# nkwangyh/CubemapSLAM

Measured on AMD Instinct MI355X. Metric: frames/sec (extract+match+localBA) on Lafida cam0, higher is better.
Workload: dtype u8 (extract/match), f64 (BA)

## Files before the change

### cubemapslam_amd/csrc/cms_api_area.hip

```cpp
#include <mutex>
#include <vector>

static int cms_area_grid_attr(int device) {
  static std::mutex mu;
  static bool done[64] = {false};
  std::lock_guard<std::mutex> lk(mu);
  if (device >= 0 && device < 64 && !done[device]) {
    HIPCHK(hipFuncSetAttribute((const void*)k_area_grid, hipFuncAttributeMaxDynamicSharedMemorySize, (CMS_AREA_MAXKP + 1) * 8));
    done[device] = true;
  }
  return CMS_OK;
}
static int cms_area_reserve(cms_ctx* c) {
  if (c->d_area_sorted) return CMS_OK;
  if (c->g.kp_cap > CMS_AREA_MAXKP) return cms_fail(CMS_ERR_UNSUPPORTED, "frame grid: more than 16383 key points per frame");
  { const int rca = cms_area_grid_attr(c->device); if (rca) return rca; }
  const size_t B = (size_t)c->max_batch;
  HIPCHK(hipMalloc((void**)&c->d_area_sorted, B * c->g.kp_cap * sizeof(uint16_t)));
  HIPCHK(hipMalloc((void**)&c->d_area_cell_start, B * (CMS_AREA_CELLS + 1) * sizeof(int)));
  HIPCHK(hipMalloc((void**)&c->d_area_nvalid, B * sizeof(int)));
  return CMS_OK;
}

static int cms_area_tmp_reserve(cms_ctx* c, int nq) {
  if ((size_t)nq <= c->area_tmp_cap) return CMS_OK;
  if (c->d_area_tmp) hipFree(c->d_area_tmp);
  c->d_area_tmp = nullptr; c->area_tmp_cap = 0;
  const size_t cap = (size_t)nq + (size_t)nq / 4 + 1024;
  HIPCHK(hipMalloc((void**)&c->d_area_tmp, cap * CMS_AREA_TMP * sizeof(int)));
  c->area_tmp_cap = cap;
  return CMS_OK;
}
static int cms_area_bsum_reserve(cms_ctx* c, int nblk) {
  if (nblk <= c->area_bsum_cap) return CMS_OK;
  if (c->d_area_bsum) hipFree(c->d_area_bsum);
  c->d_area_bsum = nullptr; c->area_bsum_cap = 0;
  HIPCHK(hipMalloc((void**)&c->d_area_bsum, (size_t)(nblk + 64) * sizeof(int)));
  c->area_bsum_cap = nblk + 64;
  return CMS_OK;
}

extern "C" int cms_area_set_keypoints(cms_ctx* c, int b, int n, const cms_keypoint* kps) {
  if (!c || b < 0 || b >= c->max_batch || n < 0 || n > c->g.kp_cap || (n > 0 && !kps)) return cms_fail(CMS_ERR_ARG, "cms_area_set_keypoints: bad argument");
  HIPCHK(hipSetDevice(c->device));
  if (n > 0) HIPCHK(hipMemcpyAsync(c->d_kps + (size_t)b * c->g.kp_cap, kps, (size_t)n * sizeof(cms_keypoint), hipMemcpyHostToDevice, c->stream));
  HIPCHK(hipMemcpyAsync(c->d_kp_cnt + b, &n, sizeof(int), hipMemcpyHostToDevice, c->stream));
  HIPCHK(hipStreamSynchronize(c->stream));
  return CMS_OK;
}

extern "C" int cms_area_grid(cms_ctx* c, int B) {
  if (!c || B < 1 || B > c->max_batch) return cms_fail(CMS_ERR_ARG, "cms_area_grid: bad batch");
  HIPCHK(hipSetDevice(c->device));
// ... 8 lines not shown
}

extern "C" int cms_features_in_area_device(cms_ctx* c, int b, int nq, const void* d_qx, const void* d_qy, const void* d_qr, const void* d_qmin,
                                           const void* d_qmax, void* d_cnt_scratch, void* d_cand_off, void* d_cand_idx, int cap, int idx_base,
                                           void* d_total) {
  if (!c || b < 0 || b >= c->area_frames || nq < 0 || cap < 0) return cms_fail(CMS_ERR_ARG, "cms_features_in_area_device: bad argument (cms_area_grid first)");
  if (nq == 0) return CMS_OK;
  HIPCHK(hipSetDevice(c->device));
  CmsAreaArgs a;
  a.kp = (const CmsKeyPoint*)c->d_kps + (size_t)b * c->g.kp_cap;
  a.sorted_idx = c->d_area_sorted + (size_t)b * c->g.kp_cap;
  a.cell_start = c->d_area_cell_start + (size_t)b * (CMS_AREA_CELLS + 1);
  a.qx = (const float*)d_qx; a.qy = (const float*)d_qy; a.qr = (const float*)d_qr; a.qmin = (const int*)d_qmin; a.qmax = (const int*)d_qmax;
  a.q_frame = nullptr; a.kp_cap = c->g.kp_cap;
  a.nq = nq; a.F = c->g.F; a.inv = (float)(3 * CMS_AREA_G) / (float)c->g.W;
  a.cnt = (int*)d_cnt_scratch; a.off = (const int*)d_cand_off; a.idx = (int*)d_cand_idx; a.cap = cap; a.idx_base = idx_base;
  hipStream_t s = c->stream;
  {
    const int nblk = (nq + 1023) / 1024, qgrid = (nq * CMS_AREA_QL + 255) / 256;
    int rcb = cms_area_bsum_reserve(c, nblk);
    if (rcb) return rcb;
    rcb = cms_area_tmp_reserve(c, nq);
    if (rcb) return rcb;
    a.tmp = c->d_area_tmp;
    hipLaunchKernelGGL(k_area_query, dim3(qgrid), dim3(256), 0, s, a, 0);
    hipLaunchKernelGGL(k_area_blocksum, dim3(nblk), dim3(1024), 0, s, (const int*)d_cnt_scratch, nq, c->d_area_bsum);
    hipLaunchKernelGGL(k_area_scan, dim3(nblk), dim3(1024), 0, s, (const int*)d_cnt_scratch, nq, (const int*)c->d_area_bsum, (int*)d_cand_off, (int*)d_total);
    hipLaunchKernelGGL(k_area_query, dim3(qgrid), dim3(256), 0, s, a, 1);
  }
  HIPCHK(hipGetLastError());
  return CMS_OK;
}

extern "C" int cms_features_in_area_batch_device(cms_ctx* c, int nq, const void* d_qframe, const void* d_qx, const void* d_qy, const void* d_qr,
                                                 const void* d_qmin, const void* d_qmax, void* d_cnt_scratch, void* d_cand_off, void* d_cand_idx,
                                                 int cap, void* d_total) {
  if (!c || nq < 0 || cap < 0 || c->area_frames < 1 || !d_qframe) return cms_fail(CMS_ERR_ARG, "cms_features_in_area_batch_device: bad argument (cms_area_grid first)");
  if (nq == 0) return CMS_OK;
  HIPCHK(hipSetDevice(c->device));
  CmsAreaArgs a;
  a.kp = (const CmsKeyPoint*)c->d_kps; a.sorted_idx = c->d_area_sorted; a.cell_start = c->d_area_cell_start;
  a.qx = (const float*)d_qx; a.qy = (const float*)d_qy; a.qr = (const float*)d_qr; a.qmin = (const int*)d_qmin; a.qmax = (const int*)d_qmax;
  a.q_frame = (const int*)d_qframe; a.kp_cap = c->g.kp_cap;
  a.nq = nq; a.F = c->g.F; a.inv = (float)(3 * CMS_AREA_G) / (float)c->g.W;
  a.cnt = (int*)d_cnt_scratch; a.off = (const int*)d_cand_off; a.idx = (int*)d_cand_idx; a.cap = cap; a.idx_base = 0;
  hipStream_t s = c->stream;
  {
    const int nblk = (nq + 1023) / 1024, qgrid = (nq * CMS_AREA_QL + 255) / 256;
    int rcb = cms_area_bsum_reserve(c, nblk);
    if (rcb) return rcb;
    rcb = cms_area_tmp_reserve(c, nq);
    if (rcb) return rcb;
    a.tmp = c->d_area_tmp;
    hipLaunchKernelGGL(k_area_query, dim3(qgrid), dim3(256), 0, s, a, 0);
    hipLaunchKernelGGL(k_area_blocksum, dim3(nblk), dim3(1024), 0, s, (const int*)d_cnt_scratch, nq, c->d_area_bsum);
    hipLaunchKernelGGL(k_area_scan, dim3(nblk), dim3(1024), 0, s, (const int*)d_cnt_scratch, nq, (const int*)c->d_area_bsum, (int*)d_cand_off, (int*)d_total);
    hipLaunchKernelGGL(k_area_query, dim3(qgrid), dim3(256), 0, s, a, 1);
  }
  HIPCHK(hipGetLastError());
  return CMS_OK;
}

extern "C" int cms_features_in_area(cms_ctx* c, int b, int nq, const float* qx, const float* qy, const float* qr, const int* qmin, const int* qmax,
                                    int* cand_off, int* cand_idx, int cap, int* total) {
  if (!c || nq < 0 || cap < 0 || !cand_off || (nq > 0 && (!qx || !qy || !qr || !qmin || !qmax))) return cms_fail(CMS_ERR_ARG, "cms_features_in_area: bad argument");
  if (b < 0 || b >= c->area_frames) return cms_fail(CMS_ERR_ARG, "cms_features_in_area: no grid for this frame (cms_area_grid first)");
  cand_off[0] = 0;
  if (total) *total = 0;
  if (nq == 0) return CMS_OK;
  HIPCHK(hipSetDevice(c->device));
  const size_t qb = (size_t)nq * 4;
  const size_t bytes = 5 * qb + qb  + (qb + 4)  + (size_t)cap * 4 + 64;
  int rc = cms_scratch(c, bytes);
  if (rc) return rc;
  uint8_t* p = (uint8_t*)c->d_match;
// ... 20 lines not shown
```

### cubemapslam_amd/csrc/cms_api_frames.hip

```cpp
#include <chrono>
#include <thread>
#include <hip/hip_runtime.h>
#include <math.h>
#include <stdio.h>
#include <stdlib.h>
#include <string.h>
#include <algorithm>
#include <string>
#include <vector>
#include "../../include/cubemapslam_hip.h"
#include "cms_types.h"
#include "orb_pattern.inc"

static bool cms_cu_mask_from_env(uint32_t* words, int* n_words) {
  const char* v = getenv("CMS_CTX_CU_MASK");
  if (!v || !*v) return false;
  int n = 0;
  while (*v && n < 8) {
    char* end = nullptr;
    words[n++] = (uint32_t)strtoul(v, &end, 16);
    if (end == v) return false;
    v = *end == ',' ? end + 1 : end;
    if (*end && *end != ',') return false;
  }
// ... 30 lines not shown
  CmsGeom g;
  float scale[CMS_MAX_LEVELS], inv_scale[CMS_MAX_LEVELS], sigma2[CMS_MAX_LEVELS], inv_sigma2[CMS_MAX_LEVELS];
  hipStream_t stream = nullptr;
  int fstride = 0;
  size_t fish_pitch = 0;
  int lut_stride = 0, mstride = 0;
  bool have_mask = false;
  int dirty_frames = 0;
  uint8_t* d_fish = nullptr; uint32_t* d_lut = nullptr; uint8_t* d_pyr = nullptr; uint8_t* d_mask = nullptr;
  CmsResizeTab* d_tab = nullptr; float* d_pattern = nullptr;
  uint32_t* d_cand = nullptr; uint16_t* d_node = nullptr; int* d_cand_cnt = nullptr; int* d_overflow = nullptr;
  uint32_t* d_qt_out = nullptr; int* d_qt_cnt = nullptr;
  uint32_t* d_cell_cand = nullptr; int* d_cell_cnt = nullptr;
  int* d_cells_all = nullptr; int* d_cells_nz = nullptr; int n_cells_all = 0, n_cells_nz = 0;
  uint16_t* d_area_sorted = nullptr; int* d_area_cell_start = nullptr; int* d_area_nvalid = nullptr; int area_frames = 0;
  int* d_area_bsum = nullptr; int area_bsum_cap = 0;
  int* d_area_tmp = nullptr; size_t area_tmp_cap = 0;
  uint8_t* h_fish_stage = nullptr; int fish_stage_frames = 0;
  hipStream_t copy_stream = nullptr; hipEvent_t ev_upload_done = nullptr, ev_remap_done = nullptr;
  bool upload_pending = false, remap_recorded = false;
  int dist_bounds_scaled = 0;
  hipEvent_t ev_block = nullptr; int last_batch = 0;
  hipEvent_t ev_extracted = nullptr; bool extracted_recorded = false;
  uint8_t* h_stage = nullptr; size_t h_stage_bytes = 0;
  CmsKeyPoint* d_kps = nullptr; uint32_t* d_aux = nullptr; uint8_t* d_desc = nullptr; int* d_kp_cnt = nullptr;
  uint32_t* d_order = nullptr; uint32_t* d_aux_sorted = nullptr; int* d_walk_cnt = nullptr; float* d_rays = nullptr;
  void* d_match = nullptr; size_t match_bytes = 0;
  bool prof = false;
  bool desc_spatial = false;
  hipEvent_t ev[8] = {nullptr, nullptr, nullptr, nullptr, nullptr, nullptr, nullptr, nullptr};
  size_t fast_lds = 0, qt_lds = 0;
// ... 68 lines not shown
    }
    out[d].s = (short)s;
    out[d].a0 = cms_sat_short((1.f - f) * 2048);
    out[d].a1 = cms_sat_short(f * 2048);
    out[d].pad = 0;
  }
}

static size_t align_up(size_t v, size_t a) { return (v + a - 1) / a * a; }

static void cms_ctx_free(cms_ctx* c) {
  if (!c) return;
  hipSetDevice(c->device);
  void* ptrs[] = {c->d_fish, c->d_lut, c->d_pyr, c->d_mask, c->d_tab, c->d_pattern, c->d_cand, c->d_node, c->d_cand_cnt,
                  c->d_overflow, c->d_qt_out, c->d_qt_cnt, c->d_kps, c->d_aux, c->d_order, c->d_aux_sorted, c->d_desc, c->d_kp_cnt, c->d_match, c->d_cell_cand,
                  c->d_cell_cnt, c->d_cells_all, c->d_cells_nz, c->d_area_sorted, c->d_area_cell_start, c->d_area_nvalid, c->d_area_bsum, c->d_area_tmp, c->d_walk_cnt, c->d_rays};
  for (void* p : ptrs) if (p) hipFree(p);
  if (c->h_fish_stage) (void)hipHostFree(c->h_fish_stage);
  if (c->h_stage) (void)hipHostFree(c->h_stage);
  for (int i = 0; i < 8; ++i) if (c->ev[i]) hipEventDestroy(c->ev[i]);
  if (c->ev_extracted) hipEventDestroy(c->ev_extracted);
  if (c->ev_block) hipEventDestroy(c->ev_block);
  if (c->ev_upload_done) hipEventDestroy(c->ev_upload_done);
  if (c->ev_remap_done) hipEventDestroy(c->ev_remap_done);
  if (c->copy_stream) hipStreamDestroy(c->copy_stream);
  if (c->stream) hipStreamDestroy(c->stream);
  delete c;
}

extern "C" int cms_ctx_create(cms_ctx** out, int device, const cms_camera* cam, const cms_orb_params* orb, int max_batch) {
  if (!out || !cam || !orb || max_batch < 1) return cms_fail(CMS_ERR_ARG, "cms_ctx_create: bad argument");
// ... 661 lines not shown
```

### cubemapslam_amd/csrc/cms_api_tri.hip

```cpp
#include <algorithm>
#include <cmath>
#include <cstdlib>
#include <cstring>
#include <memory>
#include <mutex>
#include <vector>

namespace {
inline float tri_h_small(const float* a, const float* b, int bs) {
  float t = a[0] * b[0];
  t = t + a[1] * b[bs];
  t = t + a[2] * b[2 * bs];
  return t;
}
void tri_h_e12(const float* R1w, const float* t1w, const float* R2w, const float* t2w, float* E12) {
  float R12[9], M[9], t12[3];
  for (int r = 0; r < 3; ++r)
    for (int c = 0; c < 3; ++c) {
      double s = 0;
      for (int k = 0; k < 3; ++k) s += (double)R1w[3 * r + k] * (double)R2w[3 * c + k];
      R12[3 * r + c] = (float)(s * 1.0);
      M[3 * r + c] = (float)(s * -1.0);
    }
  for (int r = 0; r < 3; ++r) t12[r] = (float)((double)tri_h_small(M + 3 * r, t2w, 1) * 1.0 + (double)t1w[r] * 1.0);
// ... 802 lines not shown
    const int sl = job_slot[j];
    if (sl < 0 || sl >= st->maxkf || !st->used[(size_t)sl] || mp_off[j + 1] < mp_off[j]) return cms_fail(CMS_ERR_ARG, "cms_kfstore_fuse_search: bad job");
    const CmsTriKF& k = st->h_kf[(size_t)sl];
    memcpy(&pose[15 * (size_t)j], k.Rcw, 36); memcpy(&pose[15 * (size_t)j + 9], k.tcw, 12); memcpy(&pose[15 * (size_t)j + 12], k.Ow, 12);
  }
  HIPCHK(hipSetDevice(c->device));
  HIPCHK(kfstore_order_behind_puts(st));
  hipStream_t s = c->stream;
  if (!job_set0) npts = nmp;
  const size_t n4 = (size_t)nmp * 4, j4 = (size_t)njobs * 4, p4 = (size_t)npts * 4;
  auto al = [](size_t v) { return (v + 255) & ~(size_t)255; };
  size_t o = 0;
  auto take = [&](size_t bytes) { const size_t at = o; o += al(bytes); return at; };
  const size_t o_pose = take(pose.size() * 4), o_joff = take(j4 + 4), o_jslot = take(j4), o_jset = take(j4), o_src = take(n4), o_job = take(n4), o_slot = take(n4), o_skip = take(nmp),
               o_pos = take(3 * p4), o_nrm = take(3 * p4), o_min = take(p4), o_max = take(p4), o_desc = take((size_t)npts * 32), o_qx = take(n4), o_qy = take(n4), o_qr = take(n4),
               o_qmin = take(n4), o_qmax = take(n4), o_lvl = take(n4), o_cnt = take(n4), o_off = take(n4 + 4), o_tot = take(16), o_bi = take(n4), o_bd = take(n4);
  const size_t fixed = o;
  bool direct = false;
  {
    hipPointerAttribute_t a1, a2;
    if (hipPointerGetAttributes(&a1, best_idx) == hipSuccess && hipPointerGetAttributes(&a2, best_dist) == hipSuccess)
      direct = a1.type == hipMemoryTypeHost && a2.type == hipMemoryTypeHost;
    else (void)hipGetLastError();
  }
  int cap = 64 * nmp + 1024;
  for (int attempt = 0; attempt < 2; ++attempt) {
    int rc = cms_scratch(c, fixed + al((size_t)cap * 4));
    if (rc) return rc;
    uint8_t* p = (uint8_t*)c->d_match;
    const size_t o_idx = fixed;
    HIPCHK(hipMemcpyAsync(p + o_pose, pose.data(), pose.size() * 4, hipMemcpyHostToDevice, s));
// ... 8 lines not shown
    HIPCHK(hipMemcpyAsync(p + o_desc, mp_desc, (size_t)npts * 32, hipMemcpyHostToDevice, s));
    const int* src_dev = job_set0 ? (const int*)(p + o_src) : nullptr;
    hipLaunchKernelGGL(k_fuse_expand_jobs, dim3((nmp + 255) / 256), dim3(256), 0, s, nmp, njobs, (const int*)(p + o_joff), (const int*)(p + o_jslot), (int*)(p + o_job), (int*)(p + o_slot),
                       job_set0 ? (const int*)(p + o_jset) : nullptr, job_set0 ? (int*)(p + o_src) : nullptr);
    CmsFuseArgs fa;
    fa.src = src_dev;
    fa.bounds_scaled = c->dist_bounds_scaled;
    fa.pose15 = (const float*)(p + o_pose); fa.mp_frame = (const int*)(p + o_job); fa.n = nmp; fa.skip = skip ? p + o_skip : nullptr;
    fa.P = (const float*)(p + o_pos); fa.normal = (const float*)(p + o_nrm); fa.min_dist = (const float*)(p + o_min); fa.max_dist = (const float*)(p + o_max);
    fa.th = th; fa.log_scale = std::log(c->scale[1]); fa.nlevels = c->g.nlevels; fa.F = c->g.F;
    for (int l = 0; l < 16; ++l) fa.sf[l] = l < c->g.nlevels ? c->scale[l] : 0.0f;
    fa.qx = (float*)(p + o_qx); fa.qy = (float*)(p + o_qy); fa.qr = (float*)(p + o_qr); fa.qmin = (int*)(p + o_qmin); fa.qmax = (int*)(p + o_qmax);
    fa.level = (int*)(p + o_lvl);
    hipLaunchKernelGGL(k_fuse_project, dim3((nmp + 255) / 256), dim3(256), 0, s, fa);
    CmsAreaArgs a;
    a.tmp = nullptr;
    a.kp = (const CmsKeyPoint*)st->d_kp; a.sorted_idx = st->d_sorted; a.cell_start = st->d_cell_start;
    a.qx = fa.qx; a.qy = fa.qy; a.qr = fa.qr; a.qmin = fa.qmin; a.qmax = fa.qmax;
    a.q_frame = (const int*)(p + o_slot); a.kp_cap = st->maxf;
    a.nq = nmp; a.F = c->g.F; a.inv = (float)(3 * CMS_AREA_G) / (float)c->g.W;
    a.cnt = (int*)(p + o_cnt); a.off = (const int*)(p + o_off); a.idx = (int*)(p + o_idx); a.cap = cap; a.idx_base = 0;
    {
      const int nblk = (nmp + 1023) / 1024, qgrid = (nmp * CMS_AREA_QL + 255) / 256;
      rc = cms_area_bsum_reserve(c, nblk);
      if (rc) return rc;
      hipLaunchKernelGGL(k_area_query, dim3(qgrid), dim3(256), 0, s, a, 0);
      hipLaunchKernelGGL(k_area_blocksum, dim3(nblk), dim3(1024), 0, s, (const int*)(p + o_cnt), nmp, c->d_area_bsum);
      hipLaunchKernelGGL(k_area_scan, dim3(nblk), dim3(1024), 0, s, (const int*)(p + o_cnt), nmp, (const int*)c->d_area_bsum, (int*)(p + o_off), (int*)(p + o_tot));
      hipLaunchKernelGGL(k_area_query, dim3(qgrid), dim3(256), 0, s, a, 1);
    }
    CmsFuseScanArgs sa;
    sa.cap = cap; sa.src = src_dev; sa.row_slot = (const int*)(p + o_slot); sa.maxf = st->maxf;
    sa.n = nmp; sa.qx = fa.qx; sa.qy = fa.qy; sa.level = fa.level; sa.mp_desc = (const uint4*)(p + o_desc);
    sa.cand_off = (const int*)(p + o_off); sa.cand_idx = (const int*)(p + o_idx); sa.kp = (const CmsKeyPoint*)st->d_kp; sa.t_desc = (const uint4*)st->d_desc;
    for (int l = 0; l < 16; ++l) sa.inv_sigma2[l] = l < c->g.nlevels ? c->inv_sigma2[l] : 0.0f;
    sa.best_idx = direct ? best_idx : (int*)(p + o_bi); sa.best_dist = direct ? best_dist : (int*)(p + o_bd);
    hipLaunchKernelGGL(k_fuse_scan, dim3((nmp * 8 + 255) / 256), dim3(256), 0, s, sa);
    HIPCHK(hipGetLastError());
    int tot = 0;
    HIPCHK(hipMemcpyAsync(&tot, p + o_tot, sizeof(int), hipMemcpyDeviceToHost, s));
    if (!direct) {
      HIPCHK(hipMemcpyAsync(best_idx, p + o_bi, n4, hipMemcpyDeviceToHost, s));
      HIPCHK(hipMemcpyAsync(best_dist, p + o_bd, n4, hipMemcpyDeviceToHost, s));
    }
    HIPCHK(hipStreamSynchronize(s));
// ... 30 lines not shown
```

### cubemapslam_amd/csrc/cms_area_kernels.hip

```cpp
#include <hip/hip_runtime.h>
#include <stdint.h>
#include "cms_types.h"
#include "cms_area_table.h"

#define CMS_AREA_CELLS (5 * CMS_AREA_G * CMS_AREA_G)
#define CMS_AREA_MAXKP 16383

extern "C" __global__ void __launch_bounds__(1024)
k_area_grid(const CmsKeyPoint* __restrict__ kps, const int* __restrict__ kp_cnt, int kp_cap, int F, float inv,
            uint16_t* __restrict__ sorted_idx, int* __restrict__ cell_start, int* __restrict__ n_valid_out) {
  extern __shared__ uint32_t area_lds[];
  uint32_t* keys = area_lds;
  uint32_t* sorted = area_lds + (kp_cap + 1);
  __shared__ int s_nvalid;
  const int b = blockIdx.x, tid = threadIdx.x, T = blockDim.x;
  const int n = min(kp_cnt[b], min(kp_cap, CMS_AREA_MAXKP));
  const CmsKeyPoint* kp = kps + (size_t)b * kp_cap;
  if (tid == 0) s_nvalid = 0;
  __syncthreads();
  for (int i = tid; i < n; i += T) {
    const float x = kp[i].x, y = kp[i].y;
    const double fi = (double)(x / (float)F), fj = (double)(y / (float)F);
    int f = -1;
    if (fi >= 0 && fi < 1 && fj >= 1 && fj < 2) f = 1;
// ... 27 lines not shown
  }
  const int last = nv ? (int)(sorted[nv - 1] >> 14) : -1;
  for (int cc = last + 1 + tid; cc <= CMS_AREA_CELLS; cc += T) cs[cc] = nv;
  if (tid == 0) n_valid_out[b] = nv;
}

struct CmsAreaArgs {
  const CmsKeyPoint* kp;
  const uint16_t* sorted_idx;
  const int* cell_start;
  const float* qx; const float* qy; const float* qr; const int* qmin; const int* qmax;
  const int* q_frame;
  int kp_cap;
  int nq, F; float inv;
  int* cnt;
  const int* off;
  int* idx; int cap; int idx_base;
  int* tmp;
};
#define CMS_AREA_TMP 8

#define CMS_AREA_QL 8
extern "C" __global__ void __launch_bounds__(256) k_area_query(CmsAreaArgs a, int pass) {
  const int gl = threadIdx.x & (CMS_AREA_QL - 1);
  const int q = (blockIdx.x * blockDim.x + threadIdx.x) / CMS_AREA_QL;
  const int qq = q < a.nq ? q : 0;
  const float x = a.qx[qq], y = a.qy[qq], r = a.qr[qq];
  const bool live = q < a.nq && !(r < 0.0f);
  const int minLevel = a.qmin[qq], maxLevel = a.qmax[qq];
  const bool check = (minLevel > 0) || (maxLevel >= 0);
  CmsAreaRectI rc[3];
  const int base = (pass && live) ? a.off[qq] : 0;
  bool copied = false;
  if (pass && a.tmp && live) {
    const int c = a.cnt[qq];
    if (c <= CMS_AREA_TMP) {
      if (gl < c && base + gl < a.cap) a.idx[base + gl] = a.tmp[(size_t)qq * CMS_AREA_TMP + gl];
      copied = true;
    }
  }
  const int nr = (live && !copied) ? cms_area_rects(x, y, r, a.F, a.inv, rc) : 0;
  int n = 0;
  int* tmpq = (!pass && a.tmp) ? a.tmp + (size_t)qq * CMS_AREA_TMP : nullptr;
  const int fr = a.q_frame ? a.q_frame[qq] : 0;
  const CmsKeyPoint* kp = a.kp + (size_t)fr * a.kp_cap;
  const uint16_t* sorted_idx = a.sorted_idx + (size_t)fr * a.kp_cap;
  const int* cell_start = a.cell_start + (size_t)fr * (CMS_AREA_CELLS + 1);
  const int idx_base = a.idx_base + (a.q_frame ? fr * a.kp_cap : 0);
  for (int k = 0; k < 3; ++k) {
    const bool has = k < nr;
    const int x0 = has ? max(0, rc[k].x0) : 0, x1 = has ? min(CMS_AREA_G - 1, rc[k].x1) : -1;
    const int y0 = has ? max(0, rc[k].y0) : 0, y1 = has ? min(CMS_AREA_G - 1, rc[k].y1) : -1;
    const int face = has ? rc[k].face : 0;
    const int ncol = (x1 >= x0 && y1 >= y0) ? x1 - x0 + 1 : 0;
    int maxcol = ncol;
    for (int o = 32; o > 0; o >>= 1) maxcol = max(maxcol, __shfl_xor(maxcol, o));
    for (int cb = 0; cb < maxcol; cb += CMS_AREA_QL) {
      const int ix = x0 + cb + gl;
      const bool col = cb + gl < ncol;
// ... 8 lines not shown
        const int j = sorted_idx[s];
        const CmsKeyPoint p = kp[j];
        if (check) {
          if (p.octave < minLevel) continue;
          if (maxLevel >= 0 && p.octave > maxLevel) continue;
        }
        if (fabsf(p.x - x) < r && fabsf(p.y - y) < r) {
          if (nh == 0) h0 = j; else if (nh == 1) h1 = j; else if (nh == 2) h2 = j; else if (nh == 3) h3 = j;
          ++nh;
        }
      }
      int incl = nh;
#pragma unroll
      for (int o = 1; o < CMS_AREA_QL; o <<= 1) { const int t = __shfl_up(incl, o, CMS_AREA_QL); if (gl >= o) incl += t; }
      const int tot = __shfl(incl, CMS_AREA_QL - 1, CMS_AREA_QL);
      if (tmpq && nh > 0) {
        int w = n + incl - nh;
        if (w < CMS_AREA_TMP) {
          if (nh <= 4) {
            tmpq[w] = idx_base + h0;
            if (nh > 1 && w + 1 < CMS_AREA_TMP) tmpq[w + 1] = idx_base + h1;
            if (nh > 2 && w + 2 < CMS_AREA_TMP) tmpq[w + 2] = idx_base + h2;
            if (nh > 3 && w + 3 < CMS_AREA_TMP) tmpq[w + 3] = idx_base + h3;
          } else {
            for (int s = s0; s < s1 && w < CMS_AREA_TMP; ++s) {
              const int j = sorted_idx[s];
              const CmsKeyPoint p = kp[j];
              if (check && (p.octave < minLevel || (maxLevel >= 0 && p.octave > maxLevel))) continue;
              if (fabsf(p.x - x) < r && fabsf(p.y - y) < r) { tmpq[w] = idx_base + j; ++w; }
            }
          }
        }
      }
      if (pass && nh > 0) {
        int w = base + n + incl - nh;
        if (nh <= 4) {
          if (w < a.cap) a.idx[w] = idx_base + h0;
          if (nh > 1 && w + 1 < a.cap) a.idx[w + 1] = idx_base + h1;
          if (nh > 2 && w + 2 < a.cap) a.idx[w + 2] = idx_base + h2;
          if (nh > 3 && w + 3 < a.cap) a.idx[w + 3] = idx_base + h3;
        } else {
          for (int s = s0; s < s1; ++s) {
            const int j = sorted_idx[s];
            const CmsKeyPoint p = kp[j];
            if (check && (p.octave < minLevel || (maxLevel >= 0 && p.octave > maxLevel))) continue;
            if (fabsf(p.x - x) < r && fabsf(p.y - y) < r) { if (w < a.cap) a.idx[w] = idx_base + j; ++w; }
          }
        }
      }
      n += tot;
    }
  }
  if (!pass && q < a.nq && gl == 0) a.cnt[q] = n;
}

extern "C" __global__ void __launch_bounds__(1024) k_area_blocksum(const int* __restrict__ cnt, int nq, int* __restrict__ bsum) {
  __shared__ int part[16];
  const int i = blockIdx.x * 1024 + threadIdx.x, lane = threadIdx.x & 63, wv = threadIdx.x >> 6;
  int v = i < nq ? cnt[i] : 0;
  for (int o = 32; o > 0; o >>= 1) v += __shfl_xor(v, o);
  if (lane == 0) part[wv] = v;
  __syncthreads();
  if (threadIdx.x == 0) { int t = 0; for (int w = 0; w < 16; ++w) t += part[w]; bsum[blockIdx.x] = t; }
}
extern "C" __global__ void __launch_bounds__(1024) k_area_scan(const int* __restrict__ cnt, int nq, const int* __restrict__ bsum,
                                                                int* __restrict__ off, int* __restrict__ total) {
  __shared__ int part[16];
  __shared__ int s_before;
  const int tid = threadIdx.x, lane = tid & 63, wv = tid >> 6;
  int before = 0;
  for (int b = tid; b < (int)blockIdx.x; b += 1024) before += bsum[b];
  for (int o = 32; o > 0; o >>= 1) before += __shfl_xor(before, o);
  if (lane == 0) part[wv] = before;
  __syncthreads();
  if (tid == 0) { int t = 0; for (int w = 0; w < 16; ++w) t += part[w]; s_before = t; }
  __syncthreads();
  const int i = blockIdx.x * 1024 + tid;
  const int v = i < nq ? cnt[i] : 0;
  int incl = v;
#pragma unroll
  for (int o = 1; o < 64; o <<= 1) { const int t = __shfl_up(incl, o); if (lane >= o) incl += t; }
  __syncthreads();
  if (lane == 63) part[wv] = incl;
  __syncthreads();
  int wbase = 0;
  for (int w = 0; w < wv; ++w) wbase += part[w];
  const int mine = s_before + wbase + incl;
  if (i < nq) off[i + 1] = mine;
  if (i == 0) off[0] = 0;
  if (i == nq - 1 && total) *total = mine;
}
```

### cubemapslam_amd/csrc/cms_area_table.h

```cpp
#ifndef CMS_AREA_TABLE_H
#define CMS_AREA_TABLE_H
#include <stdint.h>

#define CMS_AREA_G 50
#ifdef CMS_AREA_HOST_EMU
#include <math.h>
#define AREA_TAB static const
#define AREA_FN inline
#else
#define AREA_TAB static const __device__
#define AREA_FN __device__ __forceinline__
#endif

enum { AV_A, AV_B, AV_C, AV_D,
       AV_BO, AV_DO,
       AV_AU, AV_CU,
       AV_AN, AV_CN,
       AV_COUNT };
#define AE_Z 0
#define AE_G1 1
#define AE_GG 2
#define AE_V(v) (3 + (v))
#define AE_M(v) (3 + AV_COUNT + (v))

// ... 86 lines not shown
    else if (i >= 2 && i < 3 && j >= 1 && j < 2) face = 2;
  }
  if (face < 0) return 0;
  const int cornerX = (int)x / F * F, cornerY = (int)y / F * F;
  const float xin = x - (float)cornerX, yin = y - (float)cornerY;
  const float xs = xin - r, xe = xin + r, ys = yin - r, ye = yin + r;
  const bool xu = xs < 0, xo = xe > (float)(F - 1), yu = ys < 0, yo = ye > (float)(F - 1);
  const bool xinf = !xo && !xu, yinf = !yo && !yu;
  const float Ff = (float)F;
  int v[AV_COUNT];
  v[AV_A] = (int)floorf(xs * inv); v[AV_B] = (int)floorf(xe * inv); v[AV_C] = (int)floorf(ys * inv); v[AV_D] = (int)floorf(ye * inv);
  v[AV_BO] = (int)floorf((xe - Ff) * inv); v[AV_DO] = (int)floorf((ye - Ff) * inv);
  v[AV_AU] = (int)floorf((xs + Ff) * inv); v[AV_CU] = (int)floorf((ys + Ff) * inv);
  v[AV_AN] = (int)floorf((-xs) * inv); v[AV_CN] = (int)floorf((-ys) * inv);
  const CmsAreaCase* cs;
  CmsAreaCase inside;
  if (xinf && yinf) {
    inside.n = 1;
    inside.r[0].face = (int8_t)face; inside.r[0].x0 = vA; inside.r[0].x1 = vB; inside.r[0].y0 = vC; inside.r[0].y1 = vD;
    cs = &inside;
  } else if (xinf) {
    cs = &kAreaXin[face][yo ? 0 : 1];
  } else if (yinf) {
    cs = &kAreaYin[face][xo ? 0 : 1];
  } else {
    int k;
    if (xo && yo) k = 0; else if (xu && yo) k = 1; else if (xo && yu) k = 2; else k = 3;
    cs = &kAreaCorner[face][k];
  }
  auto ev = [&](int e) -> int {
    if (e == AE_Z) return 0;
    if (e == AE_G1) return CMS_AREA_G - 1;
    if (e == AE_GG) return CMS_AREA_G;
    if (e < 3 + AV_COUNT) return v[e - 3];
    return CMS_AREA_G - v[e - 3 - AV_COUNT] - 1;
// ... 31 lines not shown
```

Baseline: 23090.

## Fuse area-query scan into count kernel via decoupled group atomics

Replaces the four-launch area query pipeline (count, blocksum, scan, fill) with two kernels. The count kernel publishes per-block sums and folds them per group with packed 64-bit atomics; the last group to finish computes the group offsets, and the fill kernel derives its per-query offsets locally. The fuse path now caches up to 8 hits per query in a preallocated buffer so most queries skip the second search. The fast path for fully-inside rectangles returns directly instead of going through a temporary case struct. This cuts kernel launches and a grid-wide scan, at the cost of relying on atomics and memory fences being correct for cross-block coordination.

```diff
diff --git a/cubemapslam_amd/csrc/cms_api_area.hip b/cubemapslam_amd/csrc/cms_api_area.hip
--- a/cubemapslam_amd/csrc/cms_api_area.hip
+++ b/cubemapslam_amd/csrc/cms_api_area.hip
@@ -22,21 +22,38 @@
   return CMS_OK;
 }
 
-static int cms_area_tmp_reserve(cms_ctx* c, int nq) {
-  if ((size_t)nq <= c->area_tmp_cap) return CMS_OK;
+static int cms_area_tmp_reserve(cms_ctx* c, size_t words) {
+  if (words <= c->area_tmp_cap) return CMS_OK;
   if (c->d_area_tmp) hipFree(c->d_area_tmp);
   c->d_area_tmp = nullptr; c->area_tmp_cap = 0;
-  const size_t cap = (size_t)nq + (size_t)nq / 4 + 1024;
-  HIPCHK(hipMalloc((void**)&c->d_area_tmp, cap * CMS_AREA_TMP * sizeof(int)));
+  const size_t cap = words + words / 4 + 8192;
+  HIPCHK(hipMalloc((void**)&c->d_area_tmp, cap * sizeof(int)));
   c->area_tmp_cap = cap;
   return CMS_OK;
 }
-static int cms_area_bsum_reserve(cms_ctx* c, int nblk) {
-  if (nblk <= c->area_bsum_cap) return CMS_OK;
-  if (c->d_area_bsum) hipFree(c->d_area_bsum);
-  c->d_area_bsum = nullptr; c->area_bsum_cap = 0;
-  HIPCHK(hipMalloc((void**)&c->d_area_bsum, (size_t)(nblk + 64) * sizeof(int)));
-  c->area_bsum_cap = nblk + 64;
+static int cms_area_csr_reserve(cms_ctx* c, int ngrp) {
+  if (ngrp <= c->area_csr_gcap) return CMS_OK;
+  if (c->d_area_csr) hipFree(c->d_area_csr);
+  c->d_area_csr = nullptr; c->area_csr_gcap = 0;
+  const int gcap = ngrp + ngrp / 4 + 8;
+  HIPCHK(hipMalloc((void**)&c->d_area_csr, cms_area_csr_words(gcap) * sizeof(int)));
+  HIPCHK(hipMemsetAsync(c->d_area_csr, 0, cms_area_csr_words(gcap) * sizeof(int), c->stream));
+  c->area_csr_gcap = gcap;
+  return CMS_OK;
+}
+static int cms_area_query_launch(cms_ctx* c, CmsAreaArgs a, int keep, int* kept, int* d_off, int* d_total) {
+  const int nblk = cms_area_csr_nblk(a.nq);
+  int rc = cms_area_csr_reserve(c, cms_area_csr_ngrp(nblk));
+  if (rc) return rc;
+  if (!kept) {
+    rc = cms_area_tmp_reserve(c, (size_t)a.nq * (size_t)keep);
+    if (rc) return rc;
+    kept = c->d_area_tmp;
+  }
+  a.tmp = kept; a.keep = keep; a.csr = c->d_area_csr; a.gcap = c->area_csr_gcap; a.off = d_off; a.total = d_total;
+  hipLaunchKernelGGL(k_area_query, dim3(nblk), dim3(CMS_AREA_WG_T), 0, c->stream, a);
+  hipLaunchKernelGGL(k_area_fill, dim3(nblk), dim3(CMS_AREA_WG_T), 0, c->stream, a);
+  HIPCHK(hipGetLastError());
   return CMS_OK;
 }
 
@@ -75,22 +92,8 @@
   a.qx = (const float*)d_qx; a.qy = (const float*)d_qy; a.qr = (const float*)d_qr; a.qmin = (const int*)d_qmin; a.qmax = (const int*)d_qmax;
   a.q_frame = nullptr; a.kp_cap = c->g.kp_cap;
   a.nq = nq; a.F = c->g.F; a.inv = (float)(3 * CMS_AREA_G) / (float)c->g.W;
-  a.cnt = (int*)d_cnt_scratch; a.off = (const int*)d_cand_off; a.idx = (int*)d_cand_idx; a.cap = cap; a.idx_base = idx_base;
-  hipStream_t s = c->stream;
-  {
-    const int nblk = (nq + 1023) / 1024, qgrid = (nq * CMS_AREA_QL + 255) / 256;
-    int rcb = cms_area_bsum_reserve(c, nblk);
-    if (rcb) return rcb;
-    rcb = cms_area_tmp_reserve(c, nq);
-    if (rcb) return rcb;
-    a.tmp = c->d_area_tmp;
-    hipLaunchKernelGGL(k_area_query, dim3(qgrid), dim3(256), 0, s, a, 0);
-    hipLaunchKernelGGL(k_area_blocksum, dim3(nblk), dim3(1024), 0, s, (const int*)d_cnt_scratch, nq, c->d_area_bsum);
-    hipLaunchKernelGGL(k_area_scan, dim3(nblk), dim3(1024), 0, s, (const int*)d_cnt_scratch, nq, (const int*)c->d_area_bsum, (int*)d_cand_off, (int*)d_total);
-    hipLaunchKernelGGL(k_area_query, dim3(qgrid), dim3(256), 0, s, a, 1);
-  }
-  HIPCHK(hipGetLastError());
-  return CMS_OK;
+  a.cnt = (int*)d_cnt_scratch; a.idx = (int*)d_cand_idx; a.cap = cap; a.idx_base = idx_base;
+  return cms_area_query_launch(c, a, CMS_AREA_KEEP_TRACK, nullptr, (int*)d_cand_off, (int*)d_total);
 }
 
 extern "C" int cms_features_in_area_batch_device(cms_ctx* c, int nq, const void* d_qframe, const void* d_qx, const void* d_qy, const void* d_qr,
@@ -104,22 +107,8 @@
   a.qx = (const float*)d_qx; a.qy = (const float*)d_qy; a.qr = (const float*)d_qr; a.qmin = (const int*)d_qmin; a.qmax = (const int*)d_qmax;
   a.q_frame = (const int*)d_qframe; a.kp_cap = c->g.kp_cap;
   a.nq = nq; a.F = c->g.F; a.inv = (float)(3 * CMS_AREA_G) / (float)c->g.W;
-  a.cnt = (int*)d_cnt_scratch; a.off = (const int*)d_cand_off; a.idx = (int*)d_cand_idx; a.cap = cap; a.idx_base = 0;
-  hipStream_t s = c->stream;
-  {
-    const int nblk = (nq + 1023) / 1024, qgrid = (nq * CMS_AREA_QL + 255) / 256;
-    int rcb = cms_area_bsum_reserve(c, nblk);
-    if (rcb) return rcb;
-    rcb = cms_area_tmp_reserve(c, nq);
-    if (rcb) return rcb;
-    a.tmp = c->d_area_tmp;
-    hipLaunchKernelGGL(k_area_query, dim3(qgrid), dim3(256), 0, s, a, 0);
-    hipLaunchKernelGGL(k_area_blocksum, dim3(nblk), dim3(1024), 0, s, (const int*)d_cnt_scratch, nq, c->d_area_bsum);
-    hipLaunchKernelGGL(k_area_scan, dim3(nblk), dim3(1024), 0, s, (const int*)d_cnt_scratch, nq, (const int*)c->d_area_bsum, (int*)d_cand_off, (int*)d_total);
-    hipLaunchKernelGGL(k_area_query, dim3(qgrid), dim3(256), 0, s, a, 1);
-  }
-  HIPCHK(hipGetLastError());
-  return CMS_OK;
+  a.cnt = (int*)d_cnt_scratch; a.idx = (int*)d_cand_idx; a.cap = cap; a.idx_base = 0;
+  return cms_area_query_launch(c, a, CMS_AREA_KEEP_TRACK, nullptr, (int*)d_cand_off, (int*)d_total);
 }
 
 extern "C" int cms_features_in_area(cms_ctx* c, int b, int nq, const float* qx, const float* qy, const float* qr, const int* qmin, const int* qmax,
diff --git a/cubemapslam_amd/csrc/cms_api_frames.hip b/cubemapslam_amd/csrc/cms_api_frames.hip
--- a/cubemapslam_amd/csrc/cms_api_frames.hip
+++ b/cubemapslam_amd/csrc/cms_api_frames.hip
@@ -68,7 +68,7 @@
   uint32_t* d_cell_cand = nullptr; int* d_cell_cnt = nullptr;
   int* d_cells_all = nullptr; int* d_cells_nz = nullptr; int n_cells_all = 0, n_cells_nz = 0;
   uint16_t* d_area_sorted = nullptr; int* d_area_cell_start = nullptr; int* d_area_nvalid = nullptr; int area_frames = 0;
-  int* d_area_bsum = nullptr; int area_bsum_cap = 0;
+  int* d_area_csr = nullptr; int area_csr_gcap = 0;
   int* d_area_tmp = nullptr; size_t area_tmp_cap = 0;
   uint8_t* h_fish_stage = nullptr; int fish_stage_frames = 0;
   hipStream_t copy_stream = nullptr; hipEvent_t ev_upload_done = nullptr, ev_remap_done = nullptr;
@@ -167,7 +167,7 @@
   hipSetDevice(c->device);
   void* ptrs[] = {c->d_fish, c->d_lut, c->d_pyr, c->d_mask, c->d_tab, c->d_pattern, c->d_cand, c->d_node, c->d_cand_cnt,
                   c->d_overflow, c->d_qt_out, c->d_qt_cnt, c->d_kps, c->d_aux, c->d_order, c->d_aux_sorted, c->d_desc, c->d_kp_cnt, c->d_match, c->d_cell_cand,
-                  c->d_cell_cnt, c->d_cells_all, c->d_cells_nz, c->d_area_sorted, c->d_area_cell_start, c->d_area_nvalid, c->d_area_bsum, c->d_area_tmp, c->d_walk_cnt, c->d_rays};
+                  c->d_cell_cnt, c->d_cells_all, c->d_cells_nz, c->d_area_sorted, c->d_area_cell_start, c->d_area_nvalid, c->d_area_csr, c->d_area_tmp, c->d_walk_cnt, c->d_rays};
   for (void* p : ptrs) if (p) hipFree(p);
   if (c->h_fish_stage) (void)hipHostFree(c->h_fish_stage);
   if (c->h_stage) (void)hipHostFree(c->h_stage);
diff --git a/cubemapslam_amd/csrc/cms_api_tri.hip b/cubemapslam_amd/csrc/cms_api_tri.hip
--- a/cubemapslam_amd/csrc/cms_api_tri.hip
+++ b/cubemapslam_amd/csrc/cms_api_tri.hip
@@ -840,7 +840,7 @@
   auto take = [&](size_t bytes) { const size_t at = o; o += al(bytes); return at; };
   const size_t o_pose = take(pose.size() * 4), o_joff = take(j4 + 4), o_jslot = take(j4), o_jset = take(j4), o_src = take(n4), o_job = take(n4), o_slot = take(n4), o_skip = take(nmp),
                o_pos = take(3 * p4), o_nrm = take(3 * p4), o_min = take(p4), o_max = take(p4), o_desc = take((size_t)npts * 32), o_qx = take(n4), o_qy = take(n4), o_qr = take(n4),
-               o_qmin = take(n4), o_qmax = take(n4), o_lvl = take(n4), o_cnt = take(n4), o_off = take(n4 + 4), o_tot = take(16), o_bi = take(n4), o_bd = take(n4);
+               o_qmin = take(n4), o_qmax = take(n4), o_lvl = take(n4), o_cnt = take(n4), o_off = take(n4 + 4), o_tot = take(16), o_bi = take(n4), o_bd = take(n4), o_kept = take(n4 * CMS_AREA_KEEP_FUSE);
   const size_t fixed = o;
   bool direct = false;
   {
@@ -879,21 +879,13 @@
     fa.level = (int*)(p + o_lvl);
     hipLaunchKernelGGL(k_fuse_project, dim3((nmp + 255) / 256), dim3(256), 0, s, fa);
     CmsAreaArgs a;
-    a.tmp = nullptr;
     a.kp = (const CmsKeyPoint*)st->d_kp; a.sorted_idx = st->d_sorted; a.cell_start = st->d_cell_start;
     a.qx = fa.qx; a.qy = fa.qy; a.qr = fa.qr; a.qmin = fa.qmin; a.qmax = fa.qmax;
     a.q_frame = (const int*)(p + o_slot); a.kp_cap = st->maxf;
     a.nq = nmp; a.F = c->g.F; a.inv = (float)(3 * CMS_AREA_G) / (float)c->g.W;
-    a.cnt = (int*)(p + o_cnt); a.off = (const int*)(p + o_off); a.idx = (int*)(p + o_idx); a.cap = cap; a.idx_base = 0;
-    {
-      const int nblk = (nmp + 1023) / 1024, qgrid = (nmp * CMS_AREA_QL + 255) / 256;
-      rc = cms_area_bsum_reserve(c, nblk);
-      if (rc) return rc;
-      hipLaunchKernelGGL(k_area_query, dim3(qgrid), dim3(256), 0, s, a, 0);
-      hipLaunchKernelGGL(k_area_blocksum, dim3(nblk), dim3(1024), 0, s, (const int*)(p + o_cnt), nmp, c->d_area_bsum);
-      hipLaunchKernelGGL(k_area_scan, dim3(nblk), dim3(1024), 0, s, (const int*)(p + o_cnt), nmp, (const int*)c->d_area_bsum, (int*)(p + o_off), (int*)(p + o_tot));
-      hipLaunchKernelGGL(k_area_query, dim3(qgrid), dim3(256), 0, s, a, 1);
-    }
+    a.cnt = (int*)(p + o_cnt); a.idx = (int*)(p + o_idx); a.cap = cap; a.idx_base = 0;
+    rc = cms_area_query_launch(c, a, CMS_AREA_KEEP_FUSE, (int*)(p + o_kept), (int*)(p + o_off), (int*)(p + o_tot));
+    if (rc) return rc;
     CmsFuseScanArgs sa;
     sa.cap = cap; sa.src = src_dev; sa.row_slot = (const int*)(p + o_slot); sa.maxf = st->maxf;
     sa.n = nmp; sa.qx = fa.qx; sa.qy = fa.qy; sa.level = fa.level; sa.mp_desc = (const uint4*)(p + o_desc);
diff --git a/cubemapslam_amd/csrc/cms_area_csr.h b/cubemapslam_amd/csrc/cms_area_csr.h
--- /dev/null
+++ b/cubemapslam_amd/csrc/cms_area_csr.h
@@ -0,0 +1,44 @@
+#ifndef CMS_AREA_CSR_H
+#define CMS_AREA_CSR_H
+#include <stddef.h>
+
+#ifdef CMS_AREA_HOST_EMU
+#define AREA_CSR_FN inline
+#else
+#define AREA_CSR_FN __host__ __device__ __forceinline__
+#endif
+
+#define CMS_AREA_QL 8
+#define CMS_AREA_WG_T 256
+#define CMS_AREA_WG_Q (CMS_AREA_WG_T / CMS_AREA_QL)
+#define CMS_AREA_SCAN_T 64
+#define CMS_AREA_GRP 128
+#define CMS_AREA_CSR_HDR 16
+#define CMS_AREA_CSR_SHIFT 40
+
+AREA_CSR_FN int cms_area_csr_nblk(int nq) { return (nq + CMS_AREA_WG_Q - 1) / CMS_AREA_WG_Q; }
+AREA_CSR_FN int cms_area_csr_ngrp(int nblk) { return (nblk + CMS_AREA_GRP - 1) / CMS_AREA_GRP; }
+AREA_CSR_FN size_t cms_area_csr_words(int gcap) { return (size_t)CMS_AREA_CSR_HDR + (size_t)gcap * (4 + CMS_AREA_GRP); }
+AREA_CSR_FN int* cms_area_csr_ticket(int* scratch) { return scratch; }
+AREA_CSR_FN unsigned long long* cms_area_csr_gword(int* scratch) { return (unsigned long long*)(scratch + CMS_AREA_CSR_HDR); }
+AREA_CSR_FN int* cms_area_csr_gsum(int* scratch, int gcap) { return scratch + CMS_AREA_CSR_HDR + 2 * gcap; }
+AREA_CSR_FN int* cms_area_csr_goff(int* scratch, int gcap) { return scratch + CMS_AREA_CSR_HDR + 3 * gcap; }
+AREA_CSR_FN int* cms_area_csr_bsum(int* scratch, int gcap) { return scratch + CMS_AREA_CSR_HDR + 4 * gcap; }
+AREA_CSR_FN int cms_area_csr_group(int blk) { return blk / CMS_AREA_GRP; }
+AREA_CSR_FN int cms_area_csr_group_first(int g) { return g * CMS_AREA_GRP; }
+AREA_CSR_FN int cms_area_csr_group_size(int nblk, int g) { return nblk - g * CMS_AREA_GRP < CMS_AREA_GRP ? nblk - g * CMS_AREA_GRP : CMS_AREA_GRP; }
+AREA_CSR_FN unsigned long long cms_area_csr_pack(int sum) { return (1ull << CMS_AREA_CSR_SHIFT) | (unsigned long long)(unsigned)sum; }
+AREA_CSR_FN bool cms_area_csr_group_done(unsigned long long before, int gsize) { return (int)(before >> CMS_AREA_CSR_SHIFT) == gsize - 1; }
+AREA_CSR_FN int cms_area_csr_group_sum(unsigned long long before, int sum) { return (int)(before & ((1ull << CMS_AREA_CSR_SHIFT) - 1)) + sum; }
+AREA_CSR_FN bool cms_area_csr_is_last(int ticket_before, int ngrp) { return ticket_before == ngrp - 1; }
+AREA_CSR_FN void cms_area_csr_chunk(int ngrp, int t, int* lo, int* hi) {
+  const int per = (ngrp + CMS_AREA_SCAN_T - 1) / CMS_AREA_SCAN_T;
+  const int a = t * per < ngrp ? t * per : ngrp;
+  *lo = a;
+  *hi = a + per < ngrp ? a + per : ngrp;
+}
+AREA_CSR_FN int cms_area_csr_query(int blk, int tid) { return blk * CMS_AREA_WG_Q + tid / CMS_AREA_QL; }
+AREA_CSR_FN size_t cms_area_csr_kept(int q, int keep, int i) { return (size_t)q * (size_t)keep + (size_t)i; }
+AREA_CSR_FN bool cms_area_csr_copies(int cnt, int keep) { return cnt <= keep; }
+AREA_CSR_FN bool cms_area_csr_fits(int w, int cap) { return w < cap; }
+#endif
diff --git a/cubemapslam_amd/csrc/cms_area_kernels.hip b/cubemapslam_amd/csrc/cms_area_kernels.hip
--- a/cubemapslam_amd/csrc/cms_area_kernels.hip
+++ b/cubemapslam_amd/csrc/cms_area_kernels.hip
@@ -2,6 +2,7 @@
 #include <stdint.h>
 #include "cms_types.h"
 #include "cms_area_table.h"
+#include "cms_area_csr.h"
 
 #define CMS_AREA_CELLS (5 * CMS_AREA_G * CMS_AREA_G)
 #define CMS_AREA_MAXKP 16383
@@ -65,35 +66,29 @@
   int kp_cap;
   int nq, F; float inv;
   int* cnt;
-  const int* off;
+  int* off;
   int* idx; int cap; int idx_base;
-  int* tmp;
+  int* tmp; int keep;
+  int* csr; int gcap;
+  int* total;
 };
-#define CMS_AREA_TMP 8
-
-#define CMS_AREA_QL 8
-extern "C" __global__ void __launch_bounds__(256) k_area_query(CmsAreaArgs a, int pass) {
-  const int gl = threadIdx.x & (CMS_AREA_QL - 1);
-  const int q = (blockIdx.x * blockDim.x + threadIdx.x) / CMS_AREA_QL;
-  const int qq = q < a.nq ? q : 0;
-  const float x = a.qx[qq], y = a.qy[qq], r = a.qr[qq];
-  const bool live = q < a.nq && !(r < 0.0f);
-  const int minLevel = a.qmin[qq], maxLevel = a.qmax[qq];
+#define CMS_AREA_KEEP_TRACK 8
+#define CMS_AREA_KEEP_FUSE 8
+
+template <bool FILL>
+__device__ __forceinline__ int cms_area_search(const CmsAreaArgs& a, int qq, bool active, int gl, int base) {
+  float x = 0.0f, y = 0.0f, r = 0.0f;
+  int minLevel = -1, maxLevel = -1, fr = 0;
+  if (active) {
+    x = a.qx[qq]; y = a.qy[qq]; r = a.qr[qq]; minLevel = a.qmin[qq]; maxLevel = a.qmax[qq];
+    if (a.q_frame) fr = a.q_frame[qq];
+  }
   const bool check = (minLevel > 0) || (maxLevel >= 0);
   CmsAreaRectI rc[3];
-  const int base = (pass && live) ? a.off[qq] : 0;
-  bool copied = false;
-  if (pass && a.tmp && live) {
-    const int c = a.cnt[qq];
-    if (c <= CMS_AREA_TMP) {
-      if (gl < c && base + gl < a.cap) a.idx[base + gl] = a.tmp[(size_t)qq * CMS_AREA_TMP + gl];
-      copied = true;
-    }
-  }
-  const int nr = (live && !copied) ? cms_area_rects(x, y, r, a.F, a.inv, rc) : 0;
+  const int nr = active ? cms_area_rects(x, y, r, a.F, a.inv, rc) : 0;
   int n = 0;
-  int* tmpq = (!pass && a.tmp) ? a.tmp + (size_t)qq * CMS_AREA_TMP : nullptr;
-  const int fr = a.q_frame ? a.q_frame[qq] : 0;
+  const int keep = a.keep;
+  int* tmpq = a.tmp + cms_area_csr_kept(qq, keep, 0);
   const CmsKeyPoint* kp = a.kp + (size_t)fr * a.kp_cap;
   const uint16_t* sorted_idx = a.sorted_idx + (size_t)fr * a.kp_cap;
   const int* cell_start = a.cell_start + (size_t)fr * (CMS_AREA_CELLS + 1);
@@ -132,79 +127,123 @@
 #pragma unroll
       for (int o = 1; o < CMS_AREA_QL; o <<= 1) { const int t = __shfl_up(incl, o, CMS_AREA_QL); if (gl >= o) incl += t; }
       const int tot = __shfl(incl, CMS_AREA_QL - 1, CMS_AREA_QL);
-      if (tmpq && nh > 0) {
-        int w = n + incl - nh;
-        if (w < CMS_AREA_TMP) {
-          if (nh <= 4) {
-            tmpq[w] = idx_base + h0;
-            if (nh > 1 && w + 1 < CMS_AREA_TMP) tmpq[w + 1] = idx_base + h1;
-            if (nh > 2 && w + 2 < CMS_AREA_TMP) tmpq[w + 2] = idx_base + h2;
-            if (nh > 3 && w + 3 < CMS_AREA_TMP) tmpq[w + 3] = idx_base + h3;
-          } else {
-            for (int s = s0; s < s1 && w < CMS_AREA_TMP; ++s) {
-              const int j = sorted_idx[s];
-              const CmsKeyPoint p = kp[j];
-              if (check && (p.octave < minLevel || (maxLevel >= 0 && p.octave > maxLevel))) continue;
-              if (fabsf(p.x - x) < r && fabsf(p.y - y) < r) { tmpq[w] = idx_base + j; ++w; }
-            }
-          }
-        }
-      }
-      if (pass && nh > 0) {
-        int w = base + n + incl - nh;
+      if (nh > 0) {
+        int w = (FILL ? base : 0) + n + incl - nh;
+        const int lim = FILL ? a.cap : keep;
+        int* dst = FILL ? a.idx : tmpq;
         if (nh <= 4) {
-          if (w < a.cap) a.idx[w] = idx_base + h0;
-          if (nh > 1 && w + 1 < a.cap) a.idx[w + 1] = idx_base + h1;
-          if (nh > 2 && w + 2 < a.cap) a.idx[w + 2] = idx_base + h2;
-          if (nh > 3 && w + 3 < a.cap) a.idx[w + 3] = idx_base + h3;
+          if (w < lim) dst[w] = idx_base + h0;
+          if (nh > 1 && w + 1 < lim) dst[w + 1] = idx_base + h1;
+          if (nh > 2 && w + 2 < lim) dst[w + 2] = idx_base + h2;
+          if (nh > 3 && w + 3 < lim) dst[w + 3] = idx_base + h3;
         } else {
-          for (int s = s0; s < s1; ++s) {
+          for (int s = s0; s < s1 && w < lim; ++s) {
             const int j = sorted_idx[s];
             const CmsKeyPoint p = kp[j];
             if (check && (p.octave < minLevel || (maxLevel >= 0 && p.octave > maxLevel))) continue;
-            if (fabsf(p.x - x) < r && fabsf(p.y - y) < r) { if (w < a.cap) a.idx[w] = idx_base + j; ++w; }
+            if (fabsf(p.x - x) < r && fabsf(p.y - y) < r) { dst[w] = idx_base + j; ++w; }
           }
         }
       }
       n += tot;
     }
   }
-  if (!pass && q < a.nq && gl == 0) a.cnt[q] = n;
-}
-
-extern "C" __global__ void __launch_bounds__(1024) k_area_blocksum(const int* __restrict__ cnt, int nq, int* __restrict__ bsum) {
-  __shared__ int part[16];
-  const int i = blockIdx.x * 1024 + threadIdx.x, lane = threadIdx.x & 63, wv = threadIdx.x >> 6;
-  int v = i < nq ? cnt[i] : 0;
+  return n;
+}
+
+__device__ __forceinline__ int cms_area_wg_sum(int v, int* part) {
   for (int o = 32; o > 0; o >>= 1) v += __shfl_xor(v, o);
-  if (lane == 0) part[wv] = v;
-  __syncthreads();
-  if (threadIdx.x == 0) { int t = 0; for (int w = 0; w < 16; ++w) t += part[w]; bsum[blockIdx.x] = t; }
-}
-extern "C" __global__ void __launch_bounds__(1024) k_area_scan(const int* __restrict__ cnt, int nq, const int* __restrict__ bsum,
-                                                                int* __restrict__ off, int* __restrict__ total) {
-  __shared__ int part[16];
-  __shared__ int s_before;
-  const int tid = threadIdx.x, lane = tid & 63, wv = tid >> 6;
-  int before = 0;
-  for (int b = tid; b < (int)blockIdx.x; b += 1024) before += bsum[b];
-  for (int o = 32; o > 0; o >>= 1) before += __shfl_xor(before, o);
-  if (lane == 0) part[wv] = before;
-  __syncthreads();
-  if (tid == 0) { int t = 0; for (int w = 0; w < 16; ++w) t += part[w]; s_before = t; }
-  __syncthreads();
-  const int i = blockIdx.x * 1024 + tid;
-  const int v = i < nq ? cnt[i] : 0;
-  int incl = v;
-#pragma unroll
-  for (int o = 1; o < 64; o <<= 1) { const int t = __shfl_up(incl, o); if (lane >= o) incl += t; }
-  __syncthreads();
-  if (lane == 63) part[wv] = incl;
-  __syncthreads();
-  int wbase = 0;
-  for (int w = 0; w < wv; ++w) wbase += part[w];
-  const int mine = s_before + wbase + incl;
-  if (i < nq) off[i + 1] = mine;
-  if (i == 0) off[0] = 0;
-  if (i == nq - 1 && total) *total = mine;
-}
+  if ((threadIdx.x & 63) == 0) part[threadIdx.x >> 6] = v;
+  __syncthreads();
+  int t = 0;
+#pragma unroll
+  for (int w = 0; w < CMS_AREA_WG_T / 64; ++w) t += part[w];
+  return t;
+}
+
+extern "C" __global__ void __launch_bounds__(CMS_AREA_WG_T) k_area_query(CmsAreaArgs a) {
+  __shared__ int part[CMS_AREA_WG_T / 64];
+  const int tid = threadIdx.x, gl = tid & (CMS_AREA_QL - 1);
+  const int blk = (int)blockIdx.x, nblk = (int)gridDim.x;
+  const int q = cms_area_csr_query(blk, tid);
+  const int qq = q < a.nq ? q : 0;
+  const bool live = q < a.nq && !(a.qr[qq] < 0.0f);
+  const int n = cms_area_search<false>(a, qq, live, gl, 0);
+  if (q < a.nq && gl == 0) a.cnt[q] = n;
+  const int sum = cms_area_wg_sum((q < a.nq && gl == 0) ? n : 0, part);
+  if (tid >= 64) return;
+  const int g = cms_area_csr_group(blk), ngrp = cms_area_csr_ngrp(nblk);
+  int last = 0;
+  if (tid == 0) {
+    cms_area_csr_bsum(a.csr, a.gcap)[blk] = sum;
+    unsigned long long* gw = cms_area_csr_gword(a.csr) + g;
+    const unsigned long long before = __hip_atomic_fetch_add(gw, cms_area_csr_pack(sum), __ATOMIC_RELAXED, __HIP_MEMORY_SCOPE_AGENT);
+    if (cms_area_csr_group_done(before, cms_area_csr_group_size(nblk, g))) {
+      __hip_atomic_store(gw, 0ull, __ATOMIC_RELAXED, __HIP_MEMORY_SCOPE_AGENT);
+      __hip_atomic_store(cms_area_csr_gsum(a.csr, a.gcap) + g, cms_area_csr_group_sum(before, sum), __ATOMIC_RELAXED, __HIP_MEMORY_SCOPE_AGENT);
+      asm volatile("s_waitcnt vmcnt(0)" ::: "memory");
+      const int t = __hip_atomic_fetch_add(cms_area_csr_ticket(a.csr), 1, __ATOMIC_RELAXED, __HIP_MEMORY_SCOPE_AGENT);
+      if (cms_area_csr_is_last(t, ngrp)) {
+        __builtin_amdgcn_fence(__ATOMIC_ACQUIRE, "agent");
+        asm volatile("s_waitcnt vmcnt(0)" ::: "memory");
+        last = 1;
+      }
+    }
+  }
+  last = __shfl(last, 0);
+  if (!last) return;
+  const int* gsum = cms_area_csr_gsum(a.csr, a.gcap);
+  int lo, hi;
+  cms_area_csr_chunk(ngrp, tid, &lo, &hi);
+  int mine = 0;
+#pragma unroll 4
+  for (int b = lo; b < hi; ++b) mine += __hip_atomic_load(gsum + b, __ATOMIC_RELAXED, __HIP_MEMORY_SCOPE_AGENT);
+  int incl = mine;
+#pragma unroll
+  for (int o = 1; o < 64; o <<= 1) { const int t = __shfl_up(incl, o); if (tid >= o) incl += t; }
+  const int all = __shfl(incl, 63);
+  int run = incl - mine;
+  int* goff = cms_area_csr_goff(a.csr, a.gcap);
+#pragma unroll 4
+  for (int b = lo; b < hi; ++b) { goff[b] = run; run += __hip_atomic_load(gsum + b, __ATOMIC_RELAXED, __HIP_MEMORY_SCOPE_AGENT); }
+  if (tid == 0) {
+    a.off[0] = 0;
+    if (a.total) *a.total = all;
+    __hip_atomic_store(cms_area_csr_ticket(a.csr), 0, __ATOMIC_RELAXED, __HIP_MEMORY_SCOPE_AGENT);
+  }
+}
+
+extern "C" __global__ void __launch_bounds__(CMS_AREA_WG_T) k_area_fill(CmsAreaArgs a) {
+  __shared__ int s_off[CMS_AREA_WG_Q];
+  const int tid = threadIdx.x, gl = tid & (CMS_AREA_QL - 1);
+  const int blk = (int)blockIdx.x;
+  const int q = cms_area_csr_query(blk, tid);
+  const int qq = q < a.nq ? q : 0;
+  const int c = q < a.nq ? a.cnt[qq] : 0;
+  if (tid < 64) {
+    const int g = cms_area_csr_group(blk);
+    const int* bsum = cms_area_csr_bsum(a.csr, a.gcap);
+    int b0 = 0;
+    for (int b = cms_area_csr_group_first(g) + tid; b < blk; b += 64) b0 += bsum[b];
+    for (int o = 32; o > 0; o >>= 1) b0 += __shfl_xor(b0, o);
+    b0 += cms_area_csr_goff(a.csr, a.gcap)[g];
+    const int q2 = blk * CMS_AREA_WG_Q + tid;
+    const int v = (tid < CMS_AREA_WG_Q && q2 < a.nq) ? a.cnt[q2] : 0;
+    int incl = v;
+#pragma unroll
+    for (int o = 1; o < CMS_AREA_WG_Q; o <<= 1) { const int t = __shfl_up(incl, o); if (tid >= o) incl += t; }
+    if (tid < CMS_AREA_WG_Q) {
+      s_off[tid] = b0 + incl - v;
+      if (q2 < a.nq) a.off[q2 + 1] = b0 + incl;
+    }
+  }
+  __syncthreads();
+  const int base = s_off[tid / CMS_AREA_QL];
+  const bool copies = cms_area_csr_copies(c, a.keep);
+  if (copies) {
+    const int* tmpq = a.tmp + cms_area_csr_kept(qq, a.keep, 0);
+    for (int i = gl; i < c; i += CMS_AREA_QL)
+      if (cms_area_csr_fits(base + i, a.cap)) a.idx[base + i] = tmpq[i];
+  }
+  cms_area_search<true>(a, qq, !copies, gl, base);
+}
diff --git a/cubemapslam_amd/csrc/cms_area_table.h b/cubemapslam_amd/csrc/cms_area_table.h
--- a/cubemapslam_amd/csrc/cms_area_table.h
+++ b/cubemapslam_amd/csrc/cms_area_table.h
@@ -124,11 +124,9 @@
   v[AV_AU] = (int)floorf((xs + Ff) * inv); v[AV_CU] = (int)floorf((ys + Ff) * inv);
   v[AV_AN] = (int)floorf((-xs) * inv); v[AV_CN] = (int)floorf((-ys) * inv);
   const CmsAreaCase* cs;
-  CmsAreaCase inside;
   if (xinf && yinf) {
-    inside.n = 1;
-    inside.r[0].face = (int8_t)face; inside.r[0].x0 = vA; inside.r[0].x1 = vB; inside.r[0].y0 = vC; inside.r[0].y1 = vD;
-    cs = &inside;
+    out[0].face = face; out[0].x0 = v[AV_A]; out[0].x1 = v[AV_B]; out[0].y0 = v[AV_C]; out[0].y1 = v[AV_D];
+    return 1;
   } else if (xinf) {
     cs = &kAreaXin[face][yo ? 0 : 1];
   } else if (yinf) {
```

New measurement: 23130 (median of 3 runs). About the same (+0.2%).
